# Amandaynzhou/MMT-PSM

Hardware: AMD Instinct MI355X
Metric: imgs/sec (student+teacher step, 1000x1000, AUG_K=2) (higher is better)
Workload: dtype f32

## Files before the change

### include/mmtpsm.h

```cpp
#ifndef MMTPSM_H
#define MMTPSM_H
#include <stdint.h>
#ifdef __cplusplus
extern "C" {
#endif

#define MMT_EINVAL (-22)

int mmt_version(void);

typedef struct {
  const float* feat[4];
  float* grad_feat[4];
  int H[4];
  int W[4];
  float scale[4];
  int num_levels;
  int N;
  int C;
} mmt_pyramid;

int mmt_roi_align_forward(const mmt_pyramid* pyr , const float* rois, const int32_t* levels,
                          int K, int PH, int PW, int sampling_ratio, float* out, void* stream);
int mmt_roi_align_forward_bf16(const mmt_pyramid* pyr , const float* rois, const int32_t* levels,
// ... 66 lines not shown
                 float* out, void* stream);
int mmt_ciam_bwd(const float* x, const int64_t* group, int n, int C, int HW, int max_group, const float* gamma, const float* A,
                 const int* J, const float* dout, float* T, float* R, float* dx, float* dgamma, void* stream);
int mmt_rpn_loss(const float* obj, const float* reg, const float* labels, const float* regt, const uint8_t* pos, const uint8_t* neg,
                 long R, float beta, float* sums, float* out, float* dobj, float* dreg, void* stream);
int mmt_box_loss(const float* logits, const float* breg, const int64_t* labels, const float* regt, int R, int NC, float* out,
                 float* dlogits, float* dbreg, void* stream);
int mmt_box_loss_rows(const float* logits, const float* breg, const int64_t* labels, const float* regt, int R, int NC,
                      const int64_t* n_rows, float* out, float* dlogits, float* dbreg, void* stream);
int mmt_match_targets(const float* cand, const int32_t* cand_off, const float* gt, const int32_t* gt_off,
                      const int64_t* gt_labels, const uint8_t* visible, int N, int A_total, int G_total, int shared_cand,
                      float high, float low, int allow_low_quality, float wx, float wy, float ww, float wh, uint32_t* top_ws,
                      int32_t* matches, float* labels_f, int64_t* labels_i, float* reg, void* stream);

typedef struct {
  const float* x;
  const float* w;
  const float* scale;
  const float* shift;
  const float* res;
  const float* mask;
  const float* mul;
  float* y;
  int N, H, W, Cin, Cout, KH, KW, stride, pad, Ho, Wo;
  int relu, res_mode, out_stride, out_H, out_W;
  float mask_scale;
  const void* w_planes;
  long w_plane_stride;
  const void* x_planes;
  long x_plane_stride;
  void* y_planes;
  long y_plane_stride;
  int io_bf16;
  void* y_amax;
  const void* f16_x_amax;
  const void* f16_dy_amax;
  int y_amax_stats;
  const void* f16_guard_x;
  const void* f16_guard_dy;
  const void* w_src;
  const void* w_src_scale;
  int x_planes_layout;
  void* y_rb;
  long y_rb_stride;
  const float* y_rb_scale;
  void* y_amax_next;
  int x_planes_lag;
  int y_rb_rows;
} mmt_conv_args;

int mmt_conv_forward(const mmt_conv_args* a , void* stream);
int mmt_conv_variant(const mmt_conv_args* a );
int mmt_conv_ksplit(const mmt_conv_args* a );
int mmt_conv_wants_planes(const mmt_conv_args* a );
int mmt_set_conv_precision(int mode);
int mmt_amax(const float* x, long n, const float* rowscale, long inner, int rows, float* amax , void* stream);
int mmt_amax_stats(const float* x, long n, float* slot , void* stream);
int mmt_sum_stats(const float* a, const float* b, const float* c, const float* d, float* y, long n,
                  float* slot , void* stream);
int mmt_stats_combine(const float* const* slots , int n, float* out , void* stream);
int mmt_split_planes_f16(const float* x, void* planes, long plane_stride, long n, float scale, const float* amax ,
                         float* scale_out , float* amax_next ,
                         float* zero_slot , void* stream);
int mmt_pack_weight_f16(const float* w, void* planes, long plane_stride, int Cout, int K, float scale, const float* amax,
                        float* scale_out, void* stream);
int mmt_pack_weight_flipped_f16(const float* w, const float* scale, void* planes, long plane_stride, int Cout, int KH, int KW,
                                int Cin, const float* amax, float* scale_out, void* stream);
int mmt_conv3x3_strip_f16x2(const mmt_conv_args* a , const float* s_x , const float* s_w , void* stream);
int mmt_conv_forward_f16x2(const mmt_conv_args* a , const float* x_amax , const float* s_w , void* stream);
int mmt_get_conv_precision(void);
int mmt_stem_fused(const float* x, int N, int H, int W, const float* w_s2d, const void* w_planes, long w_plane_stride,
                   const float* s_w , const float* scale, const float* shift, const float* x_slot , float* y,
                   float* y_slot , void* stream);
int mmt_conv_wgrad_planes_splits(const mmt_conv_args* a );
int mmt_conv_wgrad_planes(const mmt_conv_args* a , const float* dy, const void* x_planes, long x_plane_stride,
                          const void* dy_planes, long dy_plane_stride, const float* s_x, const float* s_dy, const float* rowscale,
                          float* dw, float* dbias, float* workspace, void* stream);
typedef struct {
  void* fn;
  long a[16];
} mmt_call;
int mmt_replay(const mmt_call* calls , int n, int* failed_index );
int mmt_split_planes_f16_rb(const float* x, void* planes, long plane_stride, int rows, int W, int C, const float* amax,
                            float* scale_out, void* stream);
int mmt_conv_writes_rb(const mmt_conv_args* a );
typedef struct mmt_wgrad_job {
  mmt_conv_args a;
  const float* dy; const float* rowscale; float* dw; float* dbias;
  const void* x_planes; long x_plane_stride; const void* dy_planes; long dy_plane_stride; const float* s_x; const float* s_dy;
} mmt_wgrad_job;
int mmt_conv_wgrad_group_workspace(const mmt_wgrad_job* jobs , int n, long* floats_out );
int mmt_conv_wgrad_group(const mmt_wgrad_job* jobs , int n, float* workspace, long workspace_floats, void* stream);
int mmt_sum_stats_rb(const float* a, const float* b, const float* c, const float* d, float* y, int rows, int W, int C, float* slot,
                     void* planes, long plane_stride, const float* scale, float* amax_next, void* stream);
int mmt_rb_scales_update(float* state, int n, void* stream);
int mmt_conv_forward_pg(const mmt_conv_args* a , const float* s_x , const float* s_w , int tile_rows,
                        int ksplit, void* stream);
int mmt_conv_pg_plan(const mmt_conv_args* a , int* tile_rows, int* ksplit);
int mmt_conv_pg_wanted(const mmt_conv_args* a );
typedef struct { long src_off, dst_off; int Cout, K, unit0, pad; } mmt_pack_desc;
long mmt_packed_weight_elems(int Cout, int K);
int mmt_pack_weight(const float* w, void* planes, long plane_stride, int Cout, int K, void* stream);
int mmt_pack_weight_flipped(const float* w, const float* scale, void* planes, long plane_stride, int Cout, int KH, int KW,
                            int Cin, void* stream);
int mmt_split_planes(const float* x, void* planes, long plane_stride, long n, void* stream);
typedef struct { const float* w; const float* scale; void* dst; long plane_stride; int Cout, KH, KW, Cin, unit0, pad; } mmt_flip_desc;
// ... 107 lines not shown
```

### mmt-psm_amd/csrc/conv_igemm.hip

```cpp
#include <stdlib.h>
#include <map>
#include <mutex>
#include <type_traits>
#include "conv_shared.h"

namespace {

template <int BM, int BN, int WM, int WN>
__device__ __forceinline__ void conv_epilogue_stage(f32x16 (&acc)[BM / (32 * WM)][BN / (32 * WN)], float* lds,
                                                    const int lane, const int wm, const int wn) {
  constexpr int TM = BM / (32 * WM), TN = BN / (32 * WN);
  float* ct = lds;
  const int col_l = lane & 31, rq = lane >> 5;
#pragma unroll
  for (int a = 0; a < TM; a++)
#pragma unroll
    for (int b = 0; b < TN; b++)
#pragma unroll
      for (int r = 0; r < 16; r++) {
        const int row = (wm * TM + a) * 32 + (r & 3) + 8 * (r >> 2) + 4 * rq;
        ct[row * BN + (wn * TN + b) * 32 + col_l] = acc[a][b][r];
      }
}

// ... 433 lines not shown
  };

  load_tile(0);
  store_tile(0);
  __syncthreads();
  for (int kt = 0; kt < nkt; kt++) {
    const int buf = kt & 1;
    if (kt + 1 < nkt) load_tile(kt + 1);
    const char* A = ring + buf * STAGE + (wm * TM * 32) * 32 + froff;
    const char* B = ring + buf * STAGE + NS * PA + (wn * TN * 32) * 32 + froff;
    bf16x8 fa[NS][TM], fb[NS][TN];
#pragma unroll
    for (int q = 0; q < NS; q++) {
#pragma unroll
      for (int a = 0; a < TM; a++) fa[q][a] = *(const bf16x8*)(A + q * PA + a * 32 * 32);
#pragma unroll
      for (int b = 0; b < TN; b++) fb[q][b] = *(const bf16x8*)(B + q * PB + b * 32 * 32);
    }
#pragma unroll
    for (int sum = 2 * (NS - 1) > NS - 1 ? NS - 1 : 0; sum >= 0; sum--)
#pragma unroll
      for (int qa = 0; qa <= sum; qa++) {
        const int qb = sum - qa;
        if (qa < NS && qb < NS) {
#pragma unroll
          for (int a = 0; a < TM; a++)
#pragma unroll
            for (int b = 0; b < TN; b++)
              acc[a][b] = __builtin_amdgcn_mfma_f32_32x32x16_bf16(fa[qa][a], fb[qb][b], acc[a][b], 0, 0, 0);
        }
      }
    if (kt + 1 < nkt) store_tile(buf ^ 1);
    __syncthreads();
  }
  conv_epilogue<BM, BN, WM, WN>(p, acc, lds, m0, n0, tid, lane, wm, wn, HoWo);
}

__device__ __attribute__((aligned(16))) const float g_zero16[4] = {0.f, 0.f, 0.f, 0.f};

__device__ __forceinline__ void dma16(const void* g, void* l) {
  __builtin_amdgcn_global_load_lds((const __attribute__((address_space(1))) void*)g, (lds_ptr_t)l, 16, 0, 0);
}

__device__ __forceinline__ void dma16_unseen(const void* g, void* l) {
#if defined(__HIP_DEVICE_COMPILE__)
  const unsigned la = __builtin_amdgcn_readfirstlane((unsigned)(unsigned long)(__attribute__((address_space(3))) char*)l);
  asm volatile("s_mov_b32 m0, %1\n\ts_nop 0\n\tglobal_load_lds_dwordx4 %0, off" ::"v"(g), "s"(la) : "m0", "memory");
#endif
}

template <int BM, int BN, int WM, int WN, int NS, int S, bool F16 = false>
__global__ __launch_bounds__(256, 2) void conv_fwd_glds_kernel(const ConvP p, const unsigned short* __restrict__ wpl,
                                                               const long wpl_stride, const int ksplit,
                                                               float* __restrict__ ws) {
  constexpr int TM = BM / (32 * WM), TN = BN / (32 * WN);
  constexpr int A_BYTES = BM * 64;
  constexpr int PB = BN * 32;
  constexpr int STAGE = A_BYTES + NS * PB;
  constexpr int NIA = BM / 64;
  constexpr int NIB_TOT = NS * BN / 32;
  constexpr int NIB = (NIB_TOT + 3) / 4;
  constexpr int NI = NIA + NIB;
  extern __shared__ __attribute__((aligned(16))) float lds[];
  char* const ring = (char*)lds;

  const int tid = threadIdx.x;
  const int lane = tid & 63;
  const int wave = __builtin_amdgcn_readfirstlane(tid >> 6);
  const int wm = wave / WN, wn = wave % WN;

  const int tiles_m = (p.M + BM - 1) / BM;
  const int tiles_n = (p.Cout + BN - 1) / BN;
  int bid = blockIdx.x;
  {
    const int nwg = tiles_m * tiles_n * ksplit, q = nwg >> 3, r = nwg & 7, xcd = bid & 7, idx = bid >> 3;
    bid = (xcd < r ? xcd * (q + 1) : r * (q + 1) + (xcd - r) * q) + idx;
  }
  const int ks = bid % ksplit;
  bid /= ksplit;
  const int tile_m = bid / tiles_n, tile_n = bid % tiles_n;
  const int m0 = tile_m * BM, n0 = tile_n * BN;
  const int HoWo = p.Ho * p.Wo;
  F16Guard guard = {};
  if constexpr (F16) guard = f16_guard_load(p.guard_x);
  unsigned abase[NIA];
  int aih0[NIA], aiw0[NIA], achunk[NIA];
  bool aok[NIA];
#pragma unroll
  for (int i = 0; i < NIA; i++) {
    const int row = (wave + 4 * i) * 16 + (lane >> 2);
    const int m = m0 + row;
    aok[i] = m < p.M;
    const int mm = aok[i] ? m : 0;
    const int img = mm / HoWo, rem = mm - img * HoWo;
    const int ho = rem / p.Wo, wo = rem - ho * p.Wo;
    aih0[i] = ho * p.stride - p.pad;
    aiw0[i] = wo * p.stride - p.pad;
    abase[i] = (unsigned)img * (unsigned)(p.H * p.W * p.Cin);
    achunk[i] = ((lane & 3) ^ ((row >> 2) & 3)) * 4;
  }
  const int nb32 = (p.Cout + 31) >> 5;
  const long kt_stride = (long)nb32 * 512;
  const unsigned short* bsrc[NIB];
  int bdst[NIB];
#pragma unroll
  for (int i = 0; i < NIB; i++) {
    const int t = (wave + 4 * i) % NIB_TOT;
// ... 115 lines not shown
    idx -= M_RA;
    if (idx < M_RB) { const int q = idx / TN, b = idx % TN; fbn[q][b] = *(const bf16x8*)(st + boff + q * PB + b * 1024); return; }
    idx -= M_RB;
    if (idx < M_SPLIT) {
      const int lvl = idx / (2 * TM), f = idx % (2 * TM), a = f >> 1, h = f & 1;
      if (lvl & 1) split_sub(a, h); else split_cvt(a, h, lvl >> 1);
      return;
    }
    pack_a(fan);
  };
  auto wait_dma = [&](int steps_in_flight) {
    static_assert(S >= 3 && S <= 5 && 3 * NI < 64, "vmcnt range");
    if (steps_in_flight <= 0) asm volatile("s_waitcnt vmcnt(0) lgkmcnt(0)" ::: "memory");
    else if (steps_in_flight == 1) asm volatile("s_waitcnt vmcnt(%0) lgkmcnt(0)" ::"n"(NI) : "memory");
    else if (steps_in_flight == 2) asm volatile("s_waitcnt vmcnt(%0) lgkmcnt(0)" ::"n"(2 * NI) : "memory");
    else asm volatile("s_waitcnt vmcnt(%0) lgkmcnt(0)" ::"n"(3 * NI) : "memory");
  };
  auto step = [&](int kt, int stage_next, int stage_free, const bf16x8 (&fa)[NS][TM], const bf16x8 (&fb)[NS][TN],
                  bf16x8 (&fan)[NS][TM], bf16x8 (&fbn)[NS][TN]) {
    wait_dma(S - 2);
    __builtin_amdgcn_s_barrier();
    tap_next();
    filling = kt + S < nkt;
    const int kt_fill = min(kt + S, nkt - 1);
    constexpr int NM = TM * TN * (NS * (NS + 1) / 2);
    int j = 0, mi = 0;
#pragma unroll
    for (int sum = NS - 1; sum >= 0; sum--)
#pragma unroll
      for (int qa = 0; qa <= sum; qa++) {
        const int qb = sum - qa;
#pragma unroll
        for (int a = 0; a < TM; a++)
#pragma unroll
          for (int b = 0; b < TN; b++) {
            if constexpr (F16)
              acc[a][b] = __builtin_amdgcn_mfma_f32_32x32x16_f16(__builtin_bit_cast(f16x8, fa[qa][a]), __builtin_bit_cast(f16x8, fb[qb][b]), acc[a][b], 0, 0, 0);
            else
              acc[a][b] = __builtin_amdgcn_mfma_f32_32x32x16_bf16(fa[qa][a], fb[qb][b], acc[a][b], 0, 0, 0);
            j++;
#pragma unroll
            for (int r = 0; r < (NMICRO + NM - 1) / NM; r++)
              if (mi < (j * NMICRO + NM - 1) / NM) { micro(mi, kt_fill, stage_free, stage_next, fan, fbn); mi++; }
            __builtin_amdgcn_sched_barrier(0);
          }
      }
  };
#pragma unroll
  for (int t = 0; t < S - 1; t++) { filling = t < nkt; issue_all(min(t, nkt - 1), t); }
  if constexpr (F16) {
    if (f16_guard_bad(guard)) {
      asm volatile("s_waitcnt vmcnt(0)" ::: "memory");
      float* slab = ksplit > 1 ? ws + ((long)bid * ksplit + ks) * (BM * BN) : nullptr;
      conv_slow_tile(m0, BM, 0, BM, n0, BN, slab, ks != 0, tid, 256, blockIdx.x);
      return;
    }
  }
  wait_dma(S - 2);
  __builtin_amdgcn_s_barrier();
  filling = S - 1 < nkt;
  issue_all(min(S - 1, nkt - 1), S - 1);
  bf16x8 fa0[NS][TM], fb0[NS][TN], fa1[NS][TM], fb1[NS][TN];
  {
    const char* st = ring;
#pragma unroll
    for (int a = 0; a < TM; a++) { va[a][0] = *(const f32x4*)(st + aoff[a][0]); va[a][1] = *(const f32x4*)(st + aoff[a][1]); }
#pragma unroll
    for (int q = 0; q < NS; q++)
#pragma unroll
      for (int b = 0; b < TN; b++) fb0[q][b] = *(const bf16x8*)(st + boff + q * PB + b * 1024);
#pragma unroll
    for (int lvl = 0; lvl < SPL; lvl++)
#pragma unroll
      for (int f = 0; f < 2 * TM; f++) { if (lvl & 1) split_sub(f >> 1, f & 1); else split_cvt(f >> 1, f & 1, lvl >> 1); }
    pack_a(fa0);
  }
  int stage = 0;
  for (int kt = 0; kt < nkt; kt += 2) {
    const int s1 = stage == S - 1 ? 0 : stage + 1, s2 = s1 == S - 1 ? 0 : s1 + 1;
    step(kt, s1, stage, fa0, fb0, fa1, fb1);
    if (kt + 1 < nkt) step(kt + 1, s2, s1, fa1, fb1, fa0, fb0);
    stage = s2;
  }
  asm volatile("s_waitcnt vmcnt(0)" ::: "memory");
  __syncthreads();
  if (ksplit == 1) {
    if (!p.staged_epilogue && !p.io && !p.ypl && !p.mul && p.res_mode <= 1 && p.out_stride == 1 && (long)p.M * p.Cout * 4 < (1L << 31)) {
      const int mrow0 = m0 + wm * TM * 32 + 4 * (lane >> 5);
      conv_epilogue_direct<TM, TN>(p, acc, (unsigned)mrow0 * ((unsigned)p.Cout * 4u), p.M - mrow0, n0 + wn * TN * 32 + (lane & 31),
                                   (1 << (TM * TN)) - 1, lds + 64, wave, lane, tid, blockIdx.x);
      return;
    }
    conv_epilogue<BM, BN, WM, WN>(p, acc, lds, m0, n0, tid, lane, wm, wn, HoWo);
    return;
  }
  conv_epilogue_stage<BM, BN, WM, WN>(acc, lds, lane, wm, wn);
  __syncthreads();
  constexpr int TILE4 = BM * BN / 4;
  f32x4* slab = (f32x4*)ws + ((long)bid * ksplit + ks) * TILE4;
  const f32x4* ct4 = (const f32x4*)lds;
  for (int i = tid; i < TILE4; i += 256) slab[i] = ct4[i];
}

template <int BM, int BN, int WM, int WN, int NS, int S>
__global__ __launch_bounds__(256, 2) void conv_fwd_pp_kernel(const ConvP p, const int ksplit, float* __restrict__ ws) {
  constexpr int TM = BM / (32 * WM), TN = BN / (32 * WN);
  constexpr int PA = BM * 32, PB = BN * 32;
  constexpr int A_BYTES = NS * PA;
  constexpr int STAGE = A_BYTES + NS * PB;
  constexpr int NIA_TOT = NS * BM / 32, NIB_TOT = NS * BN / 32;
  constexpr int NIA = (NIA_TOT + 3) / 4, NIB = (NIB_TOT + 3) / 4, NI = NIA + NIB;
  static_assert(BM / 32 == 4 || BM / 32 == 2, "row blocks per wave");
  extern __shared__ __attribute__((aligned(16))) float lds[];
  char* const ring = (char*)lds;

  const int tid = threadIdx.x;
  const int lane = tid & 63;
  const int wave = __builtin_amdgcn_readfirstlane(tid >> 6);
  const int wm = wave / WN, wn = wave % WN;

  const int tiles_m = (p.M + BM - 1) / BM;
  const int tiles_n = (p.Cout + BN - 1) / BN;
  int bid = blockIdx.x;
  {
    const int nwg = tiles_m * tiles_n * ksplit, q = nwg >> 3, r = nwg & 7, xcd = bid & 7, idx = bid >> 3;
    bid = (xcd < r ? xcd * (q + 1) : r * (q + 1) + (xcd - r) * q) + idx;
  }
  const int ks = bid % ksplit;
  bid /= ksplit;
  const int tile_m = bid / tiles_n, tile_n = bid % tiles_n;
  const int m0 = tile_m * BM, n0 = tile_n * BN;
  const int HoWo = p.Ho * p.Wo;

  const unsigned short* asrc[NIA];
  int adst[NIA];
  int arow_blk[NIA];
#pragma unroll
  for (int i = 0; i < NIA; i++) {
    const int t = (wave + 4 * i) % NIA_TOT;
    const int q = t / (BM / 32), rb = t % (BM / 32);
    asrc[i] = p.xpl + q * p.xpl_stride;
    adst[i] = q * PA + rb * 1024;
    arow_blk[i] = rb;
  }
  constexpr int NRB = (BM / 32 == 4) ? 1 : 2;
  unsigned abase[NRB];
// ... 740 lines not shown
  if ((long)p.N * p.H * p.W * p.Cin >= 0x7fffffffL || (long)p.N * p.Ho * p.Wo * p.Cout >= 0x7fffffffL ||
      (long)p.Cout * p.KH * p.KW * p.Cin >= 0x7fffffffL) return MMT_EINVAL;
  p.M = p.N * p.Ho * p.Wo;
  p.K = p.KH * p.KW * p.Cin;
  p.cin32 = (p.Cin % 32) == 0;
  p.cin4 = (p.Cin % 4) == 0;
  return 0;
}
}

namespace {

template <int BM, int BN, int WM, int WN>
int launch_fwd(const ConvP& p, hipStream_t s) {
  const int tiles = mmt_cdiv(p.M, BM) * mmt_cdiv(p.Cout, BN);
  const size_t lds = (size_t)(2 * BM * 32 + 2 * BN * 32) * sizeof(float);
  hipLaunchKernelGGL((conv_fwd_kernel<BM, BN, WM, WN>), dim3(tiles), dim3(256), lds, s, p);
  MMT_LAUNCH_CHECK();
  return 0;
}

template <int BM, int BN, int WM, int WN, int NS>
int launch_split(const ConvP& p, hipStream_t s) {
  const int tiles = mmt_cdiv(p.M, BM) * mmt_cdiv(p.Cout, BN);
  size_t ring = (size_t)2 * NS * (BM + BN) * 32, epi = (size_t)BM * BN * sizeof(float);
  hipLaunchKernelGGL((conv_fwd_split_kernel<BM, BN, WM, WN, NS>), dim3(tiles), dim3(256), ring > epi ? ring : epi, s, p);
  MMT_LAUNCH_CHECK();
  return 0;
}

}

namespace mmtconv {
SplitWs split_workspace(hipStream_t s) {
  static std::mutex mu;
  static std::map<std::pair<int, hipStream_t>, SplitWs> table;
  int dev = 0;
  if (hipGetDevice(&dev) != hipSuccess) return SplitWs{nullptr, nullptr};
  std::lock_guard<std::mutex> g(mu);
  auto it = table.find({dev, s});
  if (it != table.end()) return it->second;
  SplitWs w{nullptr, nullptr};
  if (hipMalloc((void**)&w.ws, SPLITK_WS_BYTES) != hipSuccess) return SplitWs{nullptr, nullptr};
  if (hipMalloc((void**)&w.tickets, SPLITK_TICKETS * sizeof(unsigned)) != hipSuccess ||
      hipMemset(w.tickets, 0, SPLITK_TICKETS * sizeof(unsigned)) != hipSuccess)
    return SplitWs{nullptr, nullptr};
  table[{dev, s}] = w;
  return w;
}
}

namespace {

static int pick_ksplit(const ConvP& p) {
  const char* on_env = getenv("MMT_SPLITK");
  if ((on_env && atoi(on_env) == 0) || p.Cout < 128) return 1;
  const long t128 = (long)mmt_cdiv(p.M, 128) * mmt_cdiv(p.Cout, 128);
  const int nkt = p.K >> 4;
  constexpr int tmax = 512;
  constexpr int kmin = 128;
  if (t128 >= tmax || nkt < kmin) return 1;
  int ks = (int)(512 / t128);
  if (ks > nkt / 32) ks = nkt / 32;
  if (ks > 16) ks = 16;
  return ks < 2 ? 1 : ks;
}

template <int BM, int BN, int WM, int WN, int NS, int S>
int launch_glds(const ConvP& p, hipStream_t s, int ksplit = 1) {
  const int tiles = mmt_cdiv(p.M, BM) * mmt_cdiv(p.Cout, BN) * ksplit;
  SplitWs w{nullptr, nullptr};
  if (ksplit > 1) {
    w = split_workspace(s);
    if (!w.ws || tiles > 1024) return MMT_EINVAL;
  }
  const size_t ring = (size_t)S * (BM * 64 + NS * BN * 32), epi = (size_t)BM * BN * sizeof(float);
  const size_t lds = ring > epi ? ring : epi;
  auto kern = conv_fwd_glds_kernel<BM, BN, WM, WN, NS, S>;
  if (lds > 65536) {
    static bool done = false;
    if (!done) {
      const hipError_t e = hipFuncSetAttribute((const void*)kern, hipFuncAttributeMaxDynamicSharedMemorySize, (int)lds);
      if (e != hipSuccess) return (int)e;
      done = true;
    }
  }
  hipLaunchKernelGGL(kern, dim3(tiles), dim3(256), lds, s, p, p.wpl, p.wpl_stride, ksplit, w.ws);
  MMT_LAUNCH_CHECK();
  if (ksplit > 1) {
    if constexpr (BM == 128 && BN == 128)
      launch_finish<BM, BN>(p, tiles / ksplit, ksplit, w.ws, s);
    else
      return MMT_EINVAL;
    MMT_LAUNCH_CHECK();
  }
  return 0;
}

template <int BM, int BN, int WM, int WN, int NS, int S>
int launch_pp(const ConvP& p, hipStream_t s, int ksplit = 1) {
  const int tiles = mmt_cdiv(p.M, BM) * mmt_cdiv(p.Cout, BN) * ksplit;
  SplitWs w{nullptr, nullptr};
  if (ksplit > 1) {
    w = split_workspace(s);
    if (!w.ws || tiles > 1024) return MMT_EINVAL;
  }
  const size_t ring = (size_t)S * NS * (BM + BN) * 32, epi = (size_t)BM * BN * sizeof(float);
  const size_t lds = ring > epi ? ring : epi;
  void (*kern)(const ConvP, const int, float*) = conv_fwd_pp_kernel<BM, BN, WM, WN, NS, S>;
  if (lds > 65536) {
    const hipError_t e = hipFuncSetAttribute((const void*)kern, hipFuncAttributeMaxDynamicSharedMemorySize, (int)lds);
    if (e != hipSuccess) return (int)e;
  }
  hipLaunchKernelGGL(kern, dim3(tiles), dim3(256), lds, s, p, ksplit, w.ws);
  MMT_LAUNCH_CHECK();
  if (ksplit > 1) {
    if constexpr (BM == 128 && BN == 128)
      launch_finish<BM, BN>(p, tiles / ksplit, ksplit, w.ws, s);
    else
      return MMT_EINVAL;
    MMT_LAUNCH_CHECK();
  }
  return 0;
}

static int strip_ksplit(const ConvP& p, int tw) {
  const long tiles = (long)p.N * (p.Ho * p.Wo / 256) * mmt_cdiv(p.Cout, 128);
  if (tiles >= 256) return 1;
  if (!(p.io & IO_X)) return 0;
  const char* e = getenv("MMT_SPLITK");
  if ((e && atoi(e) == 0) || p.Wo != tw || (p.Cout & 127) || tiles < 32) return 0;
  int ks = (int)((256 + tiles - 1) / tiles);
  const int pairs = 3 * (p.Cin >> 4) / 2;
  if (ks > pairs / 3) ks = pairs / 3;
  if (ks > 8) ks = 8;
  if (tiles * ks > 512) ks = (int)(512 / tiles);
  return ks >= 2 ? ks : 0;
}

static int strip_korder(const ConvP& p) {
  int g = 4;
  while (g > 1 && ((p.Cin >> 4) % g) != 0) g >>= 1;
  return g << 24;
}

static int strip_tw(const ConvP& p, bool need_planes = true) {
// ... 36 lines not shown
  return 0;
}

static int rows_ppb(const ConvP& p) {
  const int tiles_m = mmt_cdiv(p.M, 128), npanel = mmt_cdiv(p.Cout, 32);
  if (tiles_m >= 512) return npanel;
  int groups = mmt_cdiv(512, tiles_m);
  if (groups > npanel) groups = npanel;
  return mmt_cdiv(npanel, groups);
}

template <int KT, int NS, bool F16 = false, bool MASK = false>
int launch_rows(const ConvP& p, hipStream_t s) {
  const size_t lds = 2 * (size_t)KT * NS * 1024;
  auto kern = conv1x1_rows_kernel<KT, NS, F16, MASK>;
  if (lds > 65536) {
    static bool done = false;
    if (!done) {
      const hipError_t e = hipFuncSetAttribute((const void*)kern, hipFuncAttributeMaxDynamicSharedMemorySize, (int)lds);
      if (e != hipSuccess) return (int)e;
      done = true;
    }
  }
  const int ppb = rows_ppb(p);
  hipLaunchKernelGGL(kern, dim3(mmt_cdiv(p.M, 128), mmt_cdiv(mmt_cdiv(p.Cout, 32), ppb)), dim3(256), lds, s, p, p.wpl, p.wpl_stride, ppb);
  MMT_LAUNCH_CHECK();
  return 0;
}

static bool rows_shape(const ConvP& p, bool f16) {
  const char* rows_env = getenv("MMT_ROWS");
  const int rows = rows_env ? atoi(rows_env) : 1;
  constexpr int rows_min = 256;
  constexpr int rows_min16 = 16;
  if (!rows || p.io || p.KH != 1 || p.KW != 1 || p.stride != 1 || p.pad != 0 || p.Cout < 64 || (p.Cout & 3) || p.res_mode > 2 || p.mul ||
      p.out_stride != 1 || (long)p.M * p.Cin * 4 >= (1L << 31) || (long)p.M * p.Cout * 4 >= (1L << 31) ||
      (p.res_mode == 2 && (p.Wo & 7)))
    return false;
  if (f16) return (p.Cin == 64 || p.Cin == 128 || p.Cin == 256) && p.M >= 128 * rows_min16;
  return !p.mask && p.res_mode <= 1 && (p.Cin == 64 || p.Cin == 128) && p.M >= 128 * rows_min;
}

template <int NS>
int launch_glds_variant(int variant, const ConvP& p, hipStream_t s) {
  if (rows_shape(p, false)) {
    if (p.Cin == 64) return launch_rows<4, NS>(p, s);
    if (p.Cin == 128) return launch_rows<8, NS>(p, s);
  }
  if (NS == 3) {
    const int tw = strip_tw(p);
    if (tw == 128) return launch_strip<128>(p, s);
    if (tw == 64) return launch_strip<64>(p, s);
  }
  const int ksplit = pick_ksplit(p);
  if (p.io & IO_X) {
    if constexpr (NS == 1) {
      const int tw = strip_tw(p);
      if (tw == 128) return launch_strip<128, 1>(p, s);
      if (tw == 64) return launch_strip<64, 1>(p, s);
      if (ksplit > 1) return launch_pp<128, 128, 2, 2, 1, 3>(p, s, ksplit);
      switch (variant) {
        case 1: return launch_pp<128, 128, 2, 2, 1, 3>(p, s);
        case 3: return launch_pp<128, 64, 2, 2, 1, 3>(p, s);
        default: return launch_pp<64, 64, 2, 2, 1, 3>(p, s);
      }
    }
    return MMT_EINVAL;
  }
  if (ksplit > 1) return launch_glds<128, 128, 4, 1, NS, 3>(p, s, ksplit);
  switch (variant) {
    case 1: return launch_glds<128, 128, 4, 1, NS, 3>(p, s);
    case 3: return launch_glds<128, 64, 4, 1, NS, 3>(p, s);
    default: return launch_glds<64, 64, 2, 2, NS, 3>(p, s);
  }
}

template <int NS>
int launch_split_variant(int variant, const ConvP& p, hipStream_t s) {
  switch (variant) {
    case 1: return launch_split<128, 128, 2, 2, NS>(p, s);
    case 3: return launch_split<128, 64, 2, 2, NS>(p, s);
    default: return launch_split<64, 64, 2, 2, NS>(p, s);
  }
}

}

namespace mmtconv {
static int g_precision = -1;
int precision() {
  if (g_precision < 0) {
    g_precision = getenv("MMT_CONV_PRECISION") ? atoi(getenv("MMT_CONV_PRECISION")) : 3;
    if (g_precision < 0 || g_precision > 3) g_precision = 3;
  }
  return g_precision;
}
}

extern "C" int mmt_set_conv_precision(int mode) {
  if (mode < 0 || mode > 3) return MMT_EINVAL;
  mmtconv::g_precision = mode;
  return 0;
}

extern "C" int mmt_get_conv_precision(void) { return precision(); }

extern "C" int mmt_conv3x3_strip_f16x2(const mmt_conv_args* a, const float* s_x, const float* s_w, void* stream) {
  ConvP p;
  int e = fill(p, a);
  if (e) return e;
  if (!p.y || !p.xpl || !p.wpl || !s_x || !s_w || p.io || p.ypl) return MMT_EINVAL;
  p.f16_sx = s_x; p.f16_sw = s_w;
  const int tw = strip_tw(p);
  if (!tw) return MMT_EINVAL;
  const int ksplit = strip_ksplit(p, tw);
  constexpr int NS = 2;
  hipStream_t s = (hipStream_t)stream;
  SplitWs w{nullptr, nullptr};
  if (ksplit > 1) {
    w = split_workspace(s);
    if (!w.ws) return MMT_EINVAL;
  }
// ... 3 lines not shown
    const size_t ring = (size_t)2 * (NS * R * SW * 32 + 3 * NS * 128 * 32), epi = (size_t)256 * 128 * sizeof(float);
    const size_t lds = ring > epi ? ring : epi;
    const hipError_t er = hipFuncSetAttribute((const void*)kern, hipFuncAttributeMaxDynamicSharedMemorySize, (int)lds);
    if (er != hipSuccess) return (int)er;
    hipLaunchKernelGGL(kern, dim3(tiles * ksplit), dim3(512), lds, s, p, ksplit | strip_korder(p), w.ws);
    return 0;
  };
  if (tw == 128) e = go(conv3x3_strip_kernel<128, NS, true>, 128);
  else e = go(conv3x3_strip_kernel<64, NS, true>, 64);
  if (e) return e;
  MMT_LAUNCH_CHECK();
  if (ksplit > 1) {
    launch_finish<256, 128>(p, tiles, ksplit, w.ws, s);
    MMT_LAUNCH_CHECK();
  }
  return 0;
}

static int pick_variant(const ConvP& p);
static bool rb_epilogue_ok(const ConvP& p) {
  if ((p.Cout & 15) || p.out_stride > 1 || (p.io & IO_Y) || p.mul || (long)p.M * p.Cout >= (1L << 30)) return false;
  if (c64_shape(p)) return false;
  return true;
}
extern "C" int mmt_conv_writes_rb(const mmt_conv_args* a) {
  ConvP p;
  if (fill(p, a) || precision() != 3 || p.io) return 0;
  p.f16_ax = 1;
  p.f16_sx = p.f16_sw = (const float*)16;
  return rb_epilogue_ok(p) ? 1 : 0;
}
extern "C" int mmt_conv_forward_f16x2(const mmt_conv_args* a, const float* x_amax, const float* s_w, void* stream) {
  ConvP p;
  int e = fill(p, a);
  if (e) return e;
  if (!p.y || !p.wpl || !x_amax || !s_w || p.io || p.ypl || p.xpl_rb || (p.Cin & 15) || ((size_t)p.wpl & 15) || (p.wpl_stride & 7)) return MMT_EINVAL;
  if (p.M == 0 || p.Cout == 0) return 0;
  const int variant = pick_variant(p);
  if (variant == 0) return MMT_EINVAL;
  p.f16_sx = x_amax; p.f16_sw = s_w; p.f16_ax = 1;
  hipStream_t s = (hipStream_t)stream;
  if (p.yrb && !rb_epilogue_ok(p)) return MMT_EINVAL;
  if (c64_shape(p)) return launch_c64(p, s);
  if (rows_shape(p, true)) {
    if (p.mask) {
      if (p.Cin == 64) return launch_rows<4, 2, true, true>(p, s);
      if (p.Cin == 128) return launch_rows<8, 2, true, true>(p, s);
      return launch_rows<16, 2, true, true>(p, s);
    }
    if (p.Cin == 64) return launch_rows<4, 2, true>(p, s);
    if (p.Cin == 128) return launch_rows<8, 2, true>(p, s);
    return launch_rows<16, 2, true>(p, s);
  }
  const int ksplit = pick_ksplit(p);
  constexpr int S = 3;
  auto go = [&](auto kern, int BM, int BN, int ks) -> int {
    const int tiles = mmt_cdiv(p.M, BM) * mmt_cdiv(p.Cout, BN) * ks;
    SplitWs w{nullptr, nullptr};
    if (ks > 1) {
      w = split_workspace(s);
      if (!w.ws || tiles > 1024) return MMT_EINVAL;
    }
    const size_t ring = (size_t)S * (BM * 64 + 2 * BN * 32), epi = (size_t)BM * BN * sizeof(float);
    const size_t lds = ring > epi ? ring : epi;
    if (lds > 65536) {
      const hipError_t er = hipFuncSetAttribute((const void*)kern, hipFuncAttributeMaxDynamicSharedMemorySize, (int)lds);
      if (er != hipSuccess) return (int)er;
    }
    hipLaunchKernelGGL(kern, dim3(tiles), dim3(256), lds, s, p, p.wpl, p.wpl_stride, ks, w.ws);
    if (ks > 1)
      launch_finish<128, 128>(p, tiles / ks, ks, w.ws, s);
    return 0;
  };
#define MMT_GLDS_GO(SS)                                                                                      \
  do {                                                                                                       \
    if (ksplit > 1) e = go(conv_fwd_glds_kernel<128, 128, 4, 1, 2, SS, true>, 128, 128, ksplit);            \
    else if (variant == 1) e = go(conv_fwd_glds_kernel<128, 128, 4, 1, 2, SS, true>, 128, 128, 1);          \
    else if (variant == 3) e = go(conv_fwd_glds_kernel<128, 64, 4, 1, 2, SS, true>, 128, 64, 1);            \
    else e = go(conv_fwd_glds_kernel<64, 64, 2, 2, 2, SS, true>, 64, 64, 1);                                \
  } while (0)
  MMT_GLDS_GO(3);
#undef MMT_GLDS_GO
  if (e) return e;
  MMT_LAUNCH_CHECK();
  return 0;
}

static int pick_variant(const ConvP& p) {
  if (p.Cout <= 32) return 0;
  constexpr int lowk = 256;
  constexpr int lowv = 3;
  if (p.K <= lowk) return (p.Cout >= 64 && (long)mmt_cdiv(p.M, 128) * mmt_cdiv(p.Cout, 64) >= 768) ? lowv : 2;
  const long t128 = (long)mmt_cdiv(p.M, 128) * mmt_cdiv(p.Cout, 128);
  constexpr int t128min = 256;
  if (t128 >= t128min && p.Cout > 64) return 1;
  constexpr int mid = 1;
  const long t12864 = (long)mmt_cdiv(p.M, 128) * mmt_cdiv(p.Cout, 64);
  if (mid && t12864 >= 256 && p.Cout >= 64) return 3;
  return 2;
}

extern "C" int mmt_conv_variant(const mmt_conv_args* a) {
  ConvP p;
  int e = fill(p, a);
  if (e) return e;
  const int v = pick_variant(p);
  if (v != 0 && (precision() == 3 || (precision() == 1 && (p.io & IO_X))) && strip_tw(p)) return 4;
  if (v != 0 && precision() > 0 && (p.Cin & 15) == 0 && p.wpl && pick_ksplit(p) > 1) return 1;
  return v;
}

extern "C" int mmt_conv_wants_planes(const mmt_conv_args* a) {
  ConvP p;
  int e = fill(p, a);
  if (e) return 0;
  if (precision() != 3 || pick_variant(p) == 0) return 0;
  return strip_tw(p, false) ? 1 : 0;
}

extern "C" int mmt_conv_ksplit(const mmt_conv_args* a) {
  ConvP p;
  int e = fill(p, a);
  if (e) return e;
  if (pick_variant(p) != 0 && (precision() == 3 || (precision() == 1 && (p.io & IO_X))) && strip_tw(p)) return 1;
  if (pick_variant(p) != 0 && precision() > 0 && (p.Cin & 15) == 0 && p.wpl) return pick_ksplit(p);
  return 1;
}

extern "C" int mmt_conv_forward(const mmt_conv_args* a, void* stream) {
  ConvP p;
  int e = fill(p, a);
  if (e) return e;
  if (!p.y || p.xpl_rb || p.yrb) return MMT_EINVAL;
  if (p.M == 0 || p.Cout == 0) return 0;
  hipStream_t s = (hipStream_t)stream;
  const int variant = pick_variant(p);
  const int prec = precision();
  if ((p.io & IO_X) && !(prec == 1 && variant != 0 && (p.Cin & 15) == 0 && p.wpl)) return MMT_EINVAL;
  if (!p.w && !(prec > 0 && variant != 0 && (p.Cin & 15) == 0 && p.wpl)) return MMT_EINVAL;
  if (prec > 0 && variant != 0 && (p.Cin & 15) == 0 && p.wpl) {
    if (((size_t)p.wpl & 15) || (p.wpl_stride & 7)) return MMT_EINVAL;
    if (prec == 1) return launch_glds_variant<1>(variant, p, s);
    if (prec == 2) return launch_glds_variant<2>(variant, p, s);
    return launch_glds_variant<3>(variant, p, s);
  }
  if (prec > 0 && variant != 0 && (p.Cin & 15) == 0) {
    if (prec == 1) return launch_split_variant<1>(variant, p, s);
    if (prec == 2) return launch_split_variant<2>(variant, p, s);
    return launch_split_variant<3>(variant, p, s);
  }
  switch (variant) {
    case 0: return launch_fwd<128, 32, 4, 1>(p, s);
    case 1: return launch_fwd<128, 128, 2, 2>(p, s);
    case 3: return launch_fwd<128, 64, 2, 2>(p, s);
    default: return launch_fwd<64, 64, 2, 2>(p, s);
  }
}
```

### mmt-psm_amd/maskrcnn_benchmark/_hip.py

```python
import ctypes
import weakref
import os
import threading as _threading

import torch

_HERE = os.path.dirname(os.path.abspath(__file__))
LIB_PATH = os.path.join(os.path.dirname(_HERE), "libmmtpsm.so")

c_void_p, c_int, c_float, c_double, c_int64 = ctypes.c_void_p, ctypes.c_int, ctypes.c_float, ctypes.c_double, ctypes.c_int64


class Pyramid(ctypes.Structure):
    _fields_ = [("feat", c_void_p * 4), ("grad_feat", c_void_p * 4), ("H", c_int * 4), ("W", c_int * 4),
                ("scale", c_float * 4), ("num_levels", c_int), ("N", c_int), ("C", c_int)]


class ConvArgs(ctypes.Structure):
    _fields_ = [("x", c_void_p), ("w", c_void_p), ("scale", c_void_p), ("shift", c_void_p), ("res", c_void_p),
                ("mask", c_void_p), ("mul", c_void_p), ("y", c_void_p),
                ("N", c_int), ("H", c_int), ("W", c_int), ("Cin", c_int), ("Cout", c_int), ("KH", c_int),
                ("KW", c_int), ("stride", c_int), ("pad", c_int), ("Ho", c_int), ("Wo", c_int),
                ("relu", c_int), ("res_mode", c_int), ("out_stride", c_int), ("out_H", c_int), ("out_W", c_int),
                ("mask_scale", c_float), ("w_planes", c_void_p), ("w_plane_stride", ctypes.c_long),
# ... 18 lines not shown
class RpnLevel(ctypes.Structure):
    _fields_ = [("head", c_void_p), ("anchors", c_void_p), ("topk", c_void_p), ("HW", c_int), ("k", c_int),
                ("out_off", c_int), ("pad", c_int)]


class RpnTopkLevel(ctypes.Structure):
    _fields_ = [("head", c_void_p), ("topk", c_void_p), ("HW", c_int), ("k", c_int)]


class RpnSelectArgs(ctypes.Structure):
    _fields_ = [("lv", RpnLevel * 8), ("L", c_int), ("N", c_int), ("A", c_int), ("C", c_int), ("sumk", c_int),
                ("clipv", c_float), ("lim", c_void_p), ("boxes", c_void_p), ("scores", c_void_p), ("idx", c_void_p),
                ("box_reg", c_void_p)]


class RpnPostArgs(ctypes.Structure):
    _fields_ = [("boxes", c_void_p), ("scores", c_void_p), ("idx", c_void_p), ("box_reg", c_void_p), ("keep", c_void_p),
                ("keep_cnt", c_void_p), ("seg_off", c_int * 9), ("own_pre", c_int * 8), ("L", c_int), ("N", c_int),
                ("sumk", c_int), ("kmax", c_int), ("post_n", c_int), ("fpn_post_n", c_int), ("training", c_int),
                ("cap", c_int), ("min_size_filter", c_int), ("pad", c_int), ("gt", c_void_p), ("gt_off", c_void_p),
                ("out_boxes", c_void_p), ("out_scores", c_void_p),
                ("out_idx", c_void_p), ("out_reg", c_void_p), ("out_level", c_void_p), ("out_cnt", c_void_p),
                ("key_scratch", c_void_p)]


class MgdTeachers(ctypes.Structure):
    _fields_ = [("t", c_void_p * 8), ("flip", c_int * 8), ("nt", c_int)]


class MgdStudents(ctypes.Structure):
    _fields_ = [("s", c_void_p * 4), ("mirror", c_int * 4), ("ns", c_int)]


_SIGS = {
    "mmt_version": [],
    "mmt_roi_align_forward": [ctypes.POINTER(Pyramid), c_void_p, c_void_p, c_int, c_int, c_int, c_int, c_void_p, c_void_p],
    "mmt_roi_align_forward_bf16": [ctypes.POINTER(Pyramid), c_void_p, c_void_p, c_int, c_int, c_int, c_int, c_void_p, c_void_p],
    "mmt_roi_align_backward": [ctypes.POINTER(Pyramid), c_void_p, c_void_p, c_int, c_int, c_int, c_int, c_void_p, c_void_p],
    "mmt_roi_align_backward_dense": [ctypes.POINTER(Pyramid), c_void_p, c_void_p, c_int, c_int, c_int, c_int, c_void_p, c_void_p],
    "mmt_nms_batched": [c_void_p, c_void_p, c_int, c_int, c_float, c_void_p, c_void_p, c_void_p, c_void_p],
    "mmt_resample_u8": [c_void_p, c_void_p, c_int, c_int, c_int, c_int, c_void_p, c_void_p, c_int, c_void_p],
    "mmt_aug_views": [c_void_p, c_int, c_int, c_int, c_void_p, c_void_p, c_void_p, c_void_p, c_int, ctypes.POINTER(c_float),
                      c_void_p, ctypes.c_long, c_int, c_int, c_void_p],
    "mmt_aug_erase": [c_void_p, ctypes.c_long, c_int, c_int, c_void_p, c_void_p, c_void_p, c_int, ctypes.POINTER(c_float),
                      c_void_p],
    "mmt_roi_format_levels": [c_void_p, c_void_p, c_int, c_float, c_float, c_float, c_int, c_int, c_void_p, c_void_p, c_void_p],
    "mmt_relation_reg_labels": [c_void_p, c_void_p, c_void_p, c_void_p, c_int, c_int, c_int, ctypes.POINTER(c_float), c_int, c_void_p, c_void_p],
    "mmt_match_targets": [c_void_p, c_void_p, c_void_p, c_void_p, c_void_p, c_void_p, c_int, c_int, c_int, c_int, c_float,
                          c_float, c_int, c_float, c_float, c_float, c_float, c_void_p, c_void_p, c_void_p, c_void_p, c_void_p,
                          c_void_p],
    "mmt_conv_forward": [ctypes.POINTER(ConvArgs), c_void_p],
    "mmt_conv_variant": [ctypes.POINTER(ConvArgs)],
    "mmt_conv_ksplit": [ctypes.POINTER(ConvArgs)],
    "mmt_set_conv_precision": [ctypes.c_int],
    "mmt_get_conv_precision": [],
    "mmt_pack_weight": [c_void_p, c_void_p, ctypes.c_long, c_int, c_int, c_void_p],
    "mmt_rpn_topk": [c_void_p, c_int, c_int, c_int, c_void_p, c_void_p],
    "mmt_rpn_gather_decode": [ctypes.POINTER(RpnSelectArgs), c_void_p],
    "mmt_rpn_post_select": [ctypes.POINTER(RpnPostArgs), c_void_p],
    "mmt_sample_fg_bg": [c_void_p, c_int, c_void_p, c_void_p, c_int, c_int, c_int, c_void_p, c_void_p, c_void_p, c_void_p],
    "mmt_box_decode": [c_void_p, c_void_p, c_int, c_int, c_float, c_float, c_float, c_float, c_float, c_void_p, c_void_p, c_int,
                       c_void_p, c_void_p],
    "mmt_split_planes": [c_void_p, c_void_p, ctypes.c_long, ctypes.c_long, c_void_p],
    "mmt_conv_wants_planes": [ctypes.POINTER(ConvArgs)],
    "mmt_pack_weights": [c_void_p, c_void_p, ctypes.c_long, c_void_p, c_void_p, c_int, c_void_p],
    "mmt_pack_weights_flipped": [c_void_p, c_void_p, c_int, c_void_p],
    "mmt_pack_weights_f16": [c_void_p, c_void_p, ctypes.c_long, c_void_p, c_void_p, c_int, c_int, c_void_p, c_void_p],
    "mmt_pack_weights_flipped_f16": [c_void_p, c_void_p, c_int, c_int, c_void_p, c_void_p],
    "mmt_pack_weight_flipped": [c_void_p, c_void_p, c_void_p, ctypes.c_long, c_int, c_int, c_int, c_int, c_void_p],
    "mmt_conv_wgrad_splits": [ctypes.POINTER(ConvArgs)],
    "mmt_conv_wgrad": [ctypes.POINTER(ConvArgs), c_void_p, c_void_p, c_void_p, c_void_p, c_void_p, c_void_p],
    "mmt_colsum": [c_void_p, c_int, c_int, c_void_p, c_void_p],
    "mmt_weight_flip_transpose": [c_void_p, c_void_p, c_void_p, c_int, c_int, c_int, c_int, c_void_p],
    "mmt_maxpool3x3s2": [c_void_p, c_void_p, c_int, c_int, c_int, c_int, c_int, c_int, c_void_p],
    "mmt_amax": [c_void_p, ctypes.c_long, c_void_p, ctypes.c_long, c_int, c_void_p, c_void_p],
    "mmt_amax_stats": [c_void_p, ctypes.c_long, c_void_p, c_void_p],
    "mmt_det_postprocess": [c_void_p, c_void_p, c_void_p, c_void_p, c_int, c_int, c_float, c_float, c_int, c_void_p,
                            c_void_p, c_void_p, c_void_p, c_void_p, c_void_p],
    "mmt_position_embedding": [c_void_p, c_int, c_int, c_int, c_void_p, c_void_p, c_void_p],
    "mmt_sample_fg_bg_wide": [c_void_p, c_int, c_void_p, c_void_p, c_int, c_int, c_int, c_int, c_void_p, c_void_p, c_void_p, c_void_p,
                              c_void_p],
    "mmt_rpn_loss": [c_void_p, c_void_p, c_void_p, c_void_p, c_void_p, c_void_p, ctypes.c_long, c_float, c_void_p, c_void_p, c_void_p,
                     c_void_p, c_void_p],
    "mmt_box_loss": [c_void_p, c_void_p, c_void_p, c_void_p, c_int, c_int, c_void_p, c_void_p, c_void_p, c_void_p],
    "mmt_box_loss_rows": [c_void_p, c_void_p, c_void_p, c_void_p, c_int, c_int, c_void_p, c_void_p, c_void_p, c_void_p, c_void_p],
    "mmt_relation_attention_fwd": [c_void_p, c_void_p, c_void_p, c_void_p, c_void_p, c_int, c_int, c_int, c_int, c_int, c_int, c_float,
                                   c_void_p, c_void_p, c_void_p],
    "mmt_relation_attention_bwd": [c_void_p, c_void_p, c_void_p, c_void_p, c_void_p, c_void_p, c_int, c_int, c_int, c_int, c_int, c_float,
                                   c_void_p, c_void_p, c_void_p, c_void_p, c_void_p, c_void_p],
    "mmt_ciam_fwd": [c_void_p, c_void_p, c_int, c_int, c_int, c_int, c_void_p, c_void_p, c_void_p, c_void_p, c_void_p],
    "mmt_ciam_bwd": [c_void_p, c_void_p, c_int, c_int, c_int, c_int, c_void_p, c_void_p, c_void_p, c_void_p, c_void_p, c_void_p,
                     c_void_p, c_void_p, c_void_p],
    "mmt_stats_combine": [c_void_p, c_int, c_void_p, c_void_p],
    "mmt_sum_stats": [c_void_p, c_void_p, c_void_p, c_void_p, c_void_p, ctypes.c_long, c_void_p, c_void_p],
    "mmt_split_planes_f16": [c_void_p, c_void_p, ctypes.c_long, ctypes.c_long, c_float, c_void_p, c_void_p, c_void_p, c_void_p, c_void_p],
    "mmt_split_planes_f16_rb": [c_void_p, c_void_p, ctypes.c_long, c_int, c_int, c_int, c_void_p, c_void_p, c_void_p],
    "mmt_replay": [c_void_p, c_int, c_void_p],
    "mmt_conv_writes_rb": [ctypes.POINTER(ConvArgs)],
    "mmt_conv_wgrad_group_workspace": [c_void_p, c_int, ctypes.POINTER(ctypes.c_long)],
    "mmt_conv_wgrad_group": [c_void_p, c_int, c_void_p, ctypes.c_long, c_void_p],
    "mmt_sum_stats_rb": [c_void_p, c_void_p, c_void_p, c_void_p, c_void_p, c_int, c_int, c_int, c_void_p, c_void_p, ctypes.c_long, c_void_p,
                         c_void_p, c_void_p],
    "mmt_rb_scales_update": [c_void_p, c_int, c_void_p],
    "mmt_conv_wgrad_planes_splits": [ctypes.POINTER(ConvArgs)],
    "mmt_conv_wgrad_planes": [ctypes.POINTER(ConvArgs), c_void_p, c_void_p, ctypes.c_long, c_void_p, ctypes.c_long, c_void_p, c_void_p,
                              c_void_p, c_void_p, c_void_p, c_void_p, c_void_p],
# ... 2339 lines not shown
```

Baseline: 126.6.

## Fuse split-K reduction into conv kernel via per-tile atomic tickets

```diff
diff --git a/include/mmtpsm.h b/include/mmtpsm.h
--- a/include/mmtpsm.h
+++ b/include/mmtpsm.h
@@ -142,6 +142,7 @@
 int mmt_conv_forward(const mmt_conv_args* a , void* stream);
 int mmt_conv_variant(const mmt_conv_args* a );
 int mmt_conv_ksplit(const mmt_conv_args* a );
+int mmt_conv_force_ksplit(int ksplit);
 int mmt_conv_wants_planes(const mmt_conv_args* a );
 int mmt_set_conv_precision(int mode);
 int mmt_amax(const float* x, long n, const float* rowscale, long inner, int rows, float* amax , void* stream);
diff --git a/mmt-psm_amd/csrc/conv_igemm.hip b/mmt-psm_amd/csrc/conv_igemm.hip
--- a/mmt-psm_amd/csrc/conv_igemm.hip
+++ b/mmt-psm_amd/csrc/conv_igemm.hip
@@ -509,7 +509,7 @@
 template <int BM, int BN, int WM, int WN, int NS, int S, bool F16 = false>
 __global__ __launch_bounds__(256, 2) void conv_fwd_glds_kernel(const ConvP p, const unsigned short* __restrict__ wpl,
                                                                const long wpl_stride, const int ksplit,
-                                                               float* __restrict__ ws) {
+                                                               float* __restrict__ ws, unsigned* __restrict__ tickets) {
   constexpr int TM = BM / (32 * WM), TN = BN / (32 * WN);
   constexpr int A_BYTES = BM * 64;
   constexpr int PB = BN * 32;
@@ -731,7 +731,18 @@
     if (f16_guard_bad(guard)) {
       asm volatile("s_waitcnt vmcnt(0)" ::: "memory");
       float* slab = ksplit > 1 ? ws + ((long)bid * ksplit + ks) * (BM * BN) : nullptr;
-      conv_slow_tile(m0, BM, 0, BM, n0, BN, slab, ks != 0, tid, 256, blockIdx.x);
+      bool zero = ks != 0;
+      int lin = blockIdx.x;
+      if (BM == 128 && BN == 128 && ksplit > 1 && tickets) {
+        __syncthreads();
+        unsigned* const flag = (unsigned*)lds;
+        if (tid == 0) *flag = __hip_atomic_fetch_add(tickets + bid, 1u, __ATOMIC_RELAXED, __HIP_MEMORY_SCOPE_AGENT);
+        __syncthreads();
+        if (*flag != (unsigned)(ksplit - 1)) return;
+        if (tid == 0) __hip_atomic_store(tickets + bid, 0u, __ATOMIC_RELAXED, __HIP_MEMORY_SCOPE_AGENT);
+        slab = nullptr; zero = false; lin = bid;
+      }
+      conv_slow_tile(m0, BM, 0, BM, n0, BN, slab, zero, tid, 256, lin);
       return;
     }
   }
@@ -763,14 +774,65 @@
   }
   asm volatile("s_waitcnt vmcnt(0)" ::: "memory");
   __syncthreads();
-  if (ksplit == 1) {
+  int lin = blockIdx.x;
+  if constexpr (BM == 128 && BN == 128) {
+    if (ksplit > 1 && tickets) {
+      const __amdgpu_buffer_rsrc_t rws = __builtin_amdgcn_make_buffer_rsrc((void*)ws, 0, (int)SPLITK_WS_BYTES, 0x00020000);
+      typedef unsigned u32x4 __attribute__((ext_vector_type(4)));
+      constexpr unsigned SLAB = BM * BN * 4;
+      const unsigned tile_off = (unsigned)bid * (unsigned)ksplit * SLAB + (unsigned)tid * 16u;
+      {
+        const unsigned slab_off = tile_off + (unsigned)ks * SLAB;
+#pragma unroll
+        for (int i = 0; i < TM * TN; i++)
+#pragma unroll
+          for (int r4 = 0; r4 < 4; r4++) {
+            const f32x4 v = {acc[i / TN][i % TN][4 * r4], acc[i / TN][i % TN][4 * r4 + 1], acc[i / TN][i % TN][4 * r4 + 2],
+                             acc[i / TN][i % TN][4 * r4 + 3]};
+            __builtin_amdgcn_raw_buffer_store_b128(__builtin_bit_cast(u32x4, v), rws, (int)(slab_off + (unsigned)((i * 4 + r4) * 4096)), 0, 16);
+          }
+      }
+      asm volatile("s_waitcnt vmcnt(0)" ::: "memory");
+      __syncthreads();
+      unsigned* const flag = (unsigned*)lds;
+      if (tid == 0) *flag = __hip_atomic_fetch_add(tickets + bid, 1u, __ATOMIC_RELAXED, __HIP_MEMORY_SCOPE_AGENT);
+      __syncthreads();
+      const unsigned drawn = *flag;
+      if (drawn != (unsigned)(ksplit - 1)) return;
+      __syncthreads();
+      if (tid == 0) __hip_atomic_store(tickets + bid, 0u, __ATOMIC_RELAXED, __HIP_MEMORY_SCOPE_AGENT);
+      for (int j = 0; j < ksplit; j++) {
+        const unsigned slab_off = tile_off + (unsigned)j * SLAB;
+#pragma unroll
+        for (int i = 0; i < TM * TN; i++) {
+          u32x4 t[4];
+#pragma unroll
+          for (int r4 = 0; r4 < 4; r4++) t[r4] = __builtin_amdgcn_raw_buffer_load_b128(rws, (int)(slab_off + (unsigned)((i * 4 + r4) * 4096)), 0, 16);
+#pragma unroll
+          for (int r4 = 0; r4 < 4; r4++) {
+            const f32x4 v = __builtin_bit_cast(f32x4, t[r4]);
+#pragma unroll
+            for (int c = 0; c < 4; c++) {
+              if (j == 0) acc[i / TN][i % TN][4 * r4 + c] = v[c]; else acc[i / TN][i % TN][4 * r4 + c] += v[c];
+            }
+          }
+        }
+      }
+      lin = bid;
+    }
+  }
+  if (ksplit == 1 || tickets) {
     if (!p.staged_epilogue && !p.io && !p.ypl && !p.mul && p.res_mode <= 1 && p.out_stride == 1 && (long)p.M * p.Cout * 4 < (1L << 31)) {
       const int mrow0 = m0 + wm * TM * 32 + 4 * (lane >> 5);
       conv_epilogue_direct<TM, TN>(p, acc, (unsigned)mrow0 * ((unsigned)p.Cout * 4u), p.M - mrow0, n0 + wn * TN * 32 + (lane & 31),
-                                   (1 << (TM * TN)) - 1, lds + 64, wave, lane, tid, blockIdx.x);
+                                   (1 << (TM * TN)) - 1, lds + 64, wave, lane, tid, lin);
       return;
     }
-    conv_epilogue<BM, BN, WM, WN>(p, acc, lds, m0, n0, tid, lane, wm, wn, HoWo);
+    conv_epilogue_stage<BM, BN, WM, WN>(acc, lds, lane, wm, wn);
+    __syncthreads();
+    AmaxAcc st;
+    conv_epilogue_finish<BM, BN>(p, lds, m0, n0, tid, HoWo, &st);
+    if (p.amax_out) conv_amax_commit(p, st, lin);
     return;
   }
   conv_epilogue_stage<BM, BN, WM, WN>(acc, lds, lane, wm, wn);
@@ -1617,11 +1679,15 @@
 
 namespace {
 
-static int pick_ksplit(const ConvP& p) {
+static int g_force_ksplit = 0;
+static int pick_ksplit(const ConvP& p, bool* two_launch = nullptr) {
   const char* on_env = getenv("MMT_SPLITK");
-  if ((on_env && atoi(on_env) == 0) || p.Cout < 128) return 1;
+  const int mode = on_env ? atoi(on_env) : 1;
+  if (two_launch) *two_launch = mode == 2;
+  if (mode == 0 || p.Cout < 128) return 1;
   const long t128 = (long)mmt_cdiv(p.M, 128) * mmt_cdiv(p.Cout, 128);
   const int nkt = p.K >> 4;
+  if (g_force_ksplit > 0) return (g_force_ksplit <= nkt && t128 * g_force_ksplit <= 1024) ? g_force_ksplit : 1;
   constexpr int tmax = 512;
   constexpr int kmin = 128;
   if (t128 >= tmax || nkt < kmin) return 1;
@@ -1631,13 +1697,19 @@
   return ks < 2 ? 1 : ks;
 }
 
+static bool split_fits(int tiles_times_ksplit, int ksplit) {
+  return (size_t)tiles_times_ksplit * 128 * 128 * 4 <= SPLITK_WS_BYTES && tiles_times_ksplit / ksplit <= SPLITK_TICKETS;
+}
+
 template <int BM, int BN, int WM, int WN, int NS, int S>
-int launch_glds(const ConvP& p, hipStream_t s, int ksplit = 1) {
+int launch_glds(const ConvP& p, hipStream_t s, int ksplit = 1, bool two_launch = false) {
   const int tiles = mmt_cdiv(p.M, BM) * mmt_cdiv(p.Cout, BN) * ksplit;
   SplitWs w{nullptr, nullptr};
   if (ksplit > 1) {
+    if (BM != 128 || BN != 128) return MMT_EINVAL;
     w = split_workspace(s);
-    if (!w.ws || tiles > 1024) return MMT_EINVAL;
+    if (!w.ws || !w.tickets || !split_fits(tiles, ksplit)) return MMT_EINVAL;
+    if (two_launch) w.tickets = nullptr;
   }
   const size_t ring = (size_t)S * (BM * 64 + NS * BN * 32), epi = (size_t)BM * BN * sizeof(float);
   const size_t lds = ring > epi ? ring : epi;
@@ -1650,13 +1722,10 @@
       done = true;
     }
   }
-  hipLaunchKernelGGL(kern, dim3(tiles), dim3(256), lds, s, p, p.wpl, p.wpl_stride, ksplit, w.ws);
+  hipLaunchKernelGGL(kern, dim3(tiles), dim3(256), lds, s, p, p.wpl, p.wpl_stride, ksplit, w.ws, w.tickets);
   MMT_LAUNCH_CHECK();
-  if (ksplit > 1) {
-    if constexpr (BM == 128 && BN == 128)
-      launch_finish<BM, BN>(p, tiles / ksplit, ksplit, w.ws, s);
-    else
-      return MMT_EINVAL;
+  if (ksplit > 1 && two_launch) {
+    if constexpr (BM == 128 && BN == 128) launch_finish<BM, BN>(p, tiles / ksplit, ksplit, w.ws, s);
     MMT_LAUNCH_CHECK();
   }
   return 0;
@@ -1799,7 +1868,8 @@
     if (tw == 128) return launch_strip<128>(p, s);
     if (tw == 64) return launch_strip<64>(p, s);
   }
-  const int ksplit = pick_ksplit(p);
+  bool two_launch = false;
+  const int ksplit = pick_ksplit(p, &two_launch);
   if (p.io & IO_X) {
     if constexpr (NS == 1) {
       const int tw = strip_tw(p);
@@ -1814,7 +1884,7 @@
     }
     return MMT_EINVAL;
   }
-  if (ksplit > 1) return launch_glds<128, 128, 4, 1, NS, 3>(p, s, ksplit);
+  if (ksplit > 1) return launch_glds<128, 128, 4, 1, NS, 3>(p, s, ksplit, two_launch);
   switch (variant) {
     case 1: return launch_glds<128, 128, 4, 1, NS, 3>(p, s);
     case 3: return launch_glds<128, 64, 4, 1, NS, 3>(p, s);
@@ -1924,14 +1994,16 @@
     if (p.Cin == 128) return launch_rows<8, 2, true>(p, s);
     return launch_rows<16, 2, true>(p, s);
   }
-  const int ksplit = pick_ksplit(p);
+  bool two_launch = false;
+  const int ksplit = pick_ksplit(p, &two_launch);
   constexpr int S = 3;
   auto go = [&](auto kern, int BM, int BN, int ks) -> int {
     const int tiles = mmt_cdiv(p.M, BM) * mmt_cdiv(p.Cout, BN) * ks;
     SplitWs w{nullptr, nullptr};
     if (ks > 1) {
       w = split_workspace(s);
-      if (!w.ws || tiles > 1024) return MMT_EINVAL;
+      if (!w.ws || !w.tickets || !split_fits(tiles, ks)) return MMT_EINVAL;
+      if (two_launch) w.tickets = nullptr;
     }
     const size_t ring = (size_t)S * (BM * 64 + 2 * BN * 32), epi = (size_t)BM * BN * sizeof(float);
     const size_t lds = ring > epi ? ring : epi;
@@ -1939,8 +2011,8 @@
       const hipError_t er = hipFuncSetAttribute((const void*)kern, hipFuncAttributeMaxDynamicSharedMemorySize, (int)lds);
       if (er != hipSuccess) return (int)er;
     }
-    hipLaunchKernelGGL(kern, dim3(tiles), dim3(256), lds, s, p, p.wpl, p.wpl_stride, ks, w.ws);
-    if (ks > 1)
+    hipLaunchKernelGGL(kern, dim3(tiles), dim3(256), lds, s, p, p.wpl, p.wpl_stride, ks, w.ws, w.tickets);
+    if (ks > 1 && two_launch)
       launch_finish<128, 128>(p, tiles / ks, ks, w.ws, s);
     return 0;
   };
@@ -1997,6 +2069,12 @@
   if (pick_variant(p) != 0 && (precision() == 3 || (precision() == 1 && (p.io & IO_X))) && strip_tw(p)) return 1;
   if (pick_variant(p) != 0 && precision() > 0 && (p.Cin & 15) == 0 && p.wpl) return pick_ksplit(p);
   return 1;
+}
+
+extern "C" int mmt_conv_force_ksplit(int ksplit) {
+  if (ksplit < 0 || ksplit > 64) return MMT_EINVAL;
+  g_force_ksplit = ksplit;
+  return 0;
 }
 
 extern "C" int mmt_conv_forward(const mmt_conv_args* a, void* stream) {
diff --git a/mmt-psm_amd/maskrcnn_benchmark/_hip.py b/mmt-psm_amd/maskrcnn_benchmark/_hip.py
--- a/mmt-psm_amd/maskrcnn_benchmark/_hip.py
+++ b/mmt-psm_amd/maskrcnn_benchmark/_hip.py
@@ -94,6 +94,7 @@
     "mmt_conv_forward": [ctypes.POINTER(ConvArgs), c_void_p],
     "mmt_conv_variant": [ctypes.POINTER(ConvArgs)],
     "mmt_conv_ksplit": [ctypes.POINTER(ConvArgs)],
+    "mmt_conv_force_ksplit": [ctypes.c_int],
     "mmt_set_conv_precision": [ctypes.c_int],
     "mmt_get_conv_precision": [],
     "mmt_pack_weight": [c_void_p, c_void_p, ctypes.c_long, c_int, c_int, c_void_p],
```

Result: faster. 128.1 (median of 5 runs) (+1.2%).
